# annalam/seqkit

Measured on AMD Instinct MI355X. Metric: M reads/s demultiplex (150bp, 96 barcodes) at 1/8 GPUs; % HBM roofline, higher is better.
Workload: dtype u8

## Files before the change

### seqkit_amd/build.py

```python
from __future__ import annotations

import os
import shutil
import subprocess
import sys

ROOT = os.path.dirname(os.path.abspath(__file__))
REPO = os.path.dirname(ROOT)
CSRC = os.path.join(ROOT, "csrc")
LIBDIR = os.path.join(ROOT, "lib")
BINDIR = os.path.join(ROOT, "bin")
LIB_PATH = os.path.join(LIBDIR, "libseqkit_hip.so")

HIP_SOURCES = ["sk_kernels.hip", "sk_census.hip", "sk_inflate.hip", "sk_deflate.hip", "sk_bamtext.hip", "sk_bamwrite.hip", "sk_bamminimize.hip", "sk_bammarkdup.hip", "sk_bamsubsample.hip", "sk_bammerge.hip", "sk_bamcoverage.hip", "sk_bampair.hip", "sk_bamtarget.hip", "sk_capi.hip", "sk_bamfile.cpp", "sk_bamfile_reads.cpp", "sk_bamfile_out.cpp", "sk_bamfile_coverage.cpp", "sk_lut.cpp"]
HIP_DEPS = HIP_SOURCES + ["sk_internal.h", "sk_lut.h", "sk_bamblock.h", "sk_bamfmt.h", "sk_bamfile.h", "sk_passmem.h", "sk_hoststage.h", os.path.join(REPO, "include", "seqkit_hip.h")]
HIP_FLAGS = ["--offload-arch=gfx950", "-O3", "-std=c++17", "-fPIC", "-shared", "-Wall", "-Wno-unused-function"]


def library_inputs_digest() -> str:
    import hashlib
    h = hashlib.sha256()
    h.update(" ".join(HIP_FLAGS).encode())
    for d in HIP_DEPS:
        p = d if os.path.isabs(d) else os.path.join(CSRC, d)
        with open(p, "rb") as f:
            h.update(os.path.basename(p).encode() + b"\0" + f.read())
    return h.hexdigest()[:16]


def _hipcc() -> str:
# ... 60 lines not shown
```

### seqkit_amd/csrc/sk_capi.hip

```cpp
#include <hip/hip_runtime.h>
#include <rccl/rccl.h>
#include <dlfcn.h>
#include <unistd.h>

#include <algorithm>
#include <cstdarg>
#include <cstdio>
#include <cstdlib>
#include <cstring>
#include <mutex>
#include <string>
#include <unordered_set>
#include <vector>

#include "../../include/seqkit_hip.h"
#include "sk_internal.h"
#include "sk_hoststage.h"

struct sk_ctx {
	int device = 0;
	int n_cu = 256;
	hipStream_t stream = nullptr;
	hipStream_t stream2 = nullptr;
	hipEvent_t ev0 = nullptr, ev1 = nullptr, ev_pipe = nullptr;
// ... 7 lines not shown
	int bs_bytes = 0, bs_mm_off = 0, G = 0;
	uint8_t *d_nbr = nullptr;
	sk::LutDev nbr{};
	std::vector<uint8_t> sheet;
	bool nbr_tried = false;
	int64_t nbr_keys = 0, nbr_bytes = 0;
	int detail_mode = SK_DETAIL_FULL;
	unsigned long long *d_counts = nullptr;
	unsigned long long *d_counts_wide = nullptr;
	bool wide_dirty = false;
	unsigned long long *d_count_rep = nullptr;
	int count_rep_pitch = 0;
	size_t count_rep_set = 0;
	uint8_t *ws = nullptr;
	size_t ws_bytes = 0;
	sk::ManyBatch *many_pin = nullptr;
	hipEvent_t many_ev[8] = {nullptr, nullptr, nullptr, nullptr, nullptr, nullptr, nullptr, nullptr};
	int many_next = 0;
	const void *many_no_tab = nullptr;
	int many_no_stride = 0, many_no_detail = -1;
	struct Kept { void *p = nullptr; size_t cap = 0; bool pinned = false; } kept[sk::kKeepSlots];
	void *ext = nullptr;
	void (*ext_free)(void *) = nullptr;
	sk::Census *census = nullptr;
	ncclComm_t comm = nullptr;
	int comm_ranks = 0;
	uint8_t *d_genome = nullptr;
	int64_t genome_len = 0;
	int cnt_n_chr = 0;
	int64_t cnt_n_regions = 0;
	uint8_t *d_cnt = nullptr;
	int32_t *d_chr_off = nullptr, *d_ridx = nullptr;
	uint32_t *d_rstart = nullptr, *d_rend = nullptr, *d_rpmax = nullptr, *d_region_frags = nullptr;
	int ot_n_chr = 0;
	uint8_t *d_ot = nullptr;
	int32_t *d_ot_chr_off = nullptr;
	int64_t *d_ot_rstart = nullptr, *d_ot_rpmax = nullptr;
	unsigned long long *d_ot_counters = nullptr;
};

static thread_local std::string g_create_err;

static constexpr int kManySlots = 8, kManyMax = 256;

static int fail(sk_ctx *c, int code, const char *fmt, ...)
{
	char buf[512];
	va_list ap;
	va_start(ap, fmt);
	vsnprintf(buf, sizeof buf, fmt, ap);
	va_end(ap);
	if (c) c->err = buf; else g_create_err = buf;
	return code;
}

#define SK_HIP(c, call)                                                                            \
	do {                                                                                           \
		hipError_t e_ = (call);                                                                    \
		if (e_ != hipSuccess) return fail((c), SK_ERR_HIP, "%s: %s", #call, hipGetErrorString(e_)); \
// ... 161 lines not shown
	if (!c) return;
	(void)hipSetDevice(c->device);
	if (c->stream) (void)hipStreamSynchronize(c->stream);
	if (c->stream2) (void)hipStreamSynchronize(c->stream2);
	if (c->d_raw) (void)hipFree(c->d_raw);
	if (c->d_onehot) (void)hipFree(c->d_onehot);
	if (c->d_lut) (void)hipFree(c->d_lut);
	if (c->d_bs) (void)hipFree(c->d_bs);
	if (c->d_nbr) (void)hipFree(c->d_nbr);
	if (c->d_counts) (void)hipFree(c->d_counts);
	if (c->d_counts_wide) (void)hipFree(c->d_counts_wide);
	if (c->d_count_rep) (void)hipFree(c->d_count_rep);
	if (c->ws) (void)hipFree(c->ws);
	for (auto &k : c->kept) if (k.p) { if (k.pinned) (void)hipHostFree(k.p); else (void)hipFree(k.p); }
	if (c->ext && c->ext_free) c->ext_free(c->ext);
	if (c->many_pin) (void)hipHostFree(c->many_pin);
	for (hipEvent_t e : c->many_ev) if (e) (void)hipEventDestroy(e);
	if (c->census) sk::census_destroy(c->census);
	if (c->comm) (void)sk_comm_destroy(c);
	if (c->d_cnt) (void)hipFree(c->d_cnt);
	if (c->d_ot) (void)hipFree(c->d_ot);
	if (c->d_genome) (void)hipFree(c->d_genome);
	if (c->ev0) (void)hipEventDestroy(c->ev0);
	if (c->ev1) (void)hipEventDestroy(c->ev1);
	if (c->ev_pipe) (void)hipEventDestroy(c->ev_pipe);
	if (c->stream2) (void)hipStreamDestroy(c->stream2);
	if (c->stream) (void)hipStreamDestroy(c->stream);
	delete c;
}

const char *sk_last_error(const sk_ctx *c) { return c ? c->err.c_str() : g_create_err.c_str(); }

// ... 75 lines not shown

int sk_set_barcodes(sk_ctx *c, const uint8_t *table, int S, int L, int max_diff)
{
	if (!c) return SK_ERR_INVALID;
	if (S < 0 || S > SK_MAX_SAMPLES) return fail(c, SK_ERR_INVALID, "S = %d outside 0..%d", S, SK_MAX_SAMPLES);
	if (L < 0 || L > SK_MAX_BARCODE_LEN || (S > 0 && L == 0)) return fail(c, SK_ERR_INVALID, "L = %d outside 1..%d", L, SK_MAX_BARCODE_LEN);
	if (S > 0 && !table) return fail(c, SK_ERR_INVALID, "table is NULL");
	if (max_diff < 0 || max_diff > 255) return fail(c, SK_ERR_INVALID, "max_diff = %d outside 0..255", max_diff);
	if (int r = bind(c)) return r;
	SK_HIP(c, hipStreamSynchronize(c->stream));
	if (c->d_raw) { SK_HIP(c, hipFree(c->d_raw)); c->d_raw = nullptr; }
	if (c->d_onehot) { SK_HIP(c, hipFree(c->d_onehot)); c->d_onehot = nullptr; }
	if (c->d_lut) { SK_HIP(c, hipFree(c->d_lut)); c->d_lut = nullptr; }
	if (c->d_bs) { SK_HIP(c, hipFree(c->d_bs)); c->d_bs = nullptr; }
	if (c->d_nbr) { SK_HIP(c, hipFree(c->d_nbr)); c->d_nbr = nullptr; }
	c->many_no_tab = nullptr;
	c->nbr = sk::LutDev{};
	c->bs_bytes = c->bs_mm_off = c->G = 0;
	if (c->d_counts) { SK_HIP(c, hipFree(c->d_counts)); c->d_counts = nullptr; }
	if (c->d_counts_wide) { SK_HIP(c, hipFree(c->d_counts_wide)); c->d_counts_wide = nullptr; }
	c->wide_dirty = false;
	if (c->d_count_rep) { SK_HIP(c, hipFree(c->d_count_rep)); c->d_count_rep = nullptr; }
	c->have_table = false;
	c->S = S; c->L = L; c->max_diff = max_diff;
	c->W = (L + 3) / 4;

	SK_HIP(c, hipMalloc((void **)&c->d_raw, (size_t)S * L + 16));
	if (S > 0) SK_HIP(c, hipMemcpy(c->d_raw, table, (size_t)S * L, hipMemcpyHostToDevice));

	bool onehot_ok = S > 0 && L <= sk::kMaxOneHotLen && !getenv("SK_NO_ONEHOT");
	std::vector<uint8_t> lut((size_t)(L ? L : 1) * 256, 0x80);
// ... 438 lines not shown
	if (t.bc && t.counts_wide) c->wide_dirty = true;
	SK_HIP(c, sk::launch_tile_pass(t, c->n_cu, c->stream));
	return SK_OK;
}

static void one_mate(sk_fused_args &a, const uint8_t *seq, const uint8_t *qual, const uint16_t *len, int stride, int64_t n,
                     uint8_t min_baseq, uint8_t *out_seq, uint16_t *lowest_k);

int sk_fused_pass_many_dev(sk_ctx *c, const sk_fused_args *batches, int n_batches)
{
	if (!c) return SK_ERR_INVALID;
	if (n_batches < 0 || (n_batches > 0 && !batches)) return fail(c, SK_ERR_INVALID, "n_batches = %d", n_batches);
	if (n_batches == 0) return SK_OK;
	if (int r = bind(c)) return r;
	for (int i = 0; i < n_batches; i++) if (int r = check_fused(c, &batches[i], true)) return r;
	{
		bool same = n_batches >= 2;
		int64_t rows = 0;
		for (int i = 0; i < n_batches && same; i++) {
			const sk_fused_args &a = batches[i], &f = batches[0];
			bool mates = false;
			for (int m = 0; m < a.n_mates; m++) mates = mates || a.mate[m].out_seq || a.mate[m].lowest_k;
			same = !mates && a.bc && !a.counts && a.bc_stride == f.bc_stride && !a.lowest_diff == !f.lowest_diff && !a.first_idx == !f.first_idx && !a.last_idx == !f.last_idx;
			rows += ((a.n + 255) / 256) * 256;
		}
		if (const char *ev = getenv("SK_MANY_ONE_LAUNCH")) same = same && atoi(ev) != 0;
		const int want_detail_key = same ? ((batches[0].lowest_diff ? 1 : 0) | (batches[0].first_idx ? 2 : 0) | (batches[0].last_idx ? 4 : 0) | (c->detail_mode << 3)) : 0;
		if (same && c->many_no_tab && c->many_no_tab == (const void *)c->d_nbr && c->many_no_stride == batches[0].bc_stride && c->many_no_detail == want_detail_key && !getenv("SK_LUT_MANY_GATHER")) same = false;
		if (same && rows > 0 && rows < ((int64_t)1 << 31) && n_batches <= kManyMax) {
			if (int r = prepare_demux(c, &batches[0])) return r;
			if (!c->many_pin) {
				SK_HIP(c, hipHostMalloc((void **)&c->many_pin, kManySlots * kManyMax * sizeof(sk::ManyBatch), hipHostMallocDefault));
				for (int k = 0; k < kManySlots; k++) SK_HIP(c, hipEventCreateWithFlags(&c->many_ev[k], hipEventDisableTiming));
			}
			const int slot = c->many_next++ % kManySlots;
			SK_HIP(c, hipEventSynchronize(c->many_ev[slot]));
			sk::ManyBatch *hb = c->many_pin + (size_t)slot * kManyMax;
			int64_t q0 = 0;
			int nb = 0;
			for (int i = 0; i < n_batches; i++) {
				const sk_fused_args &a = batches[i];
				if (a.n == 0) continue;
				const int64_t r0 = q0 * 256;
				sk::ManyBatch &m = hb[nb++];
				m.bc = a.bc - r0 * a.bc_stride;
				m.assign = a.assign - r0;
				m.lowest_diff = a.lowest_diff ? a.lowest_diff - r0 : nullptr;
				m.first_idx = a.first_idx ? a.first_idx - r0 : nullptr;
				m.last_idx = a.last_idx ? a.last_idx - r0 : nullptr;
				m.row_end = (uint32_t)(r0 + a.n);
				q0 += (a.n + 255) / 256;
				m.q_end = (int32_t)q0;
			}
			if (nb > 0) {
				sk_fused_args first = batches[0];
				for (int i = 0; i < n_batches; i++) if (batches[i].n > 0) { first = batches[i]; break; }
				sk::TileArgs t = tile_args_of(c, &first);
				t.n = q0 * 256;
				t.many = hb; t.n_many = nb; t.many_quads = (int)q0;
				if (t.counts_wide) c->wide_dirty = true;
				const hipError_t e = sk::launch_tile_pass(t, c->n_cu, c->stream);
				SK_HIP(c, hipEventRecord(c->many_ev[slot], c->stream));
				if (e == hipSuccess) return SK_OK;
				if (e != hipErrorNotSupported) return fail(c, SK_ERR_HIP, "launch_tile_pass (many batches): %s", hipGetErrorString(e));
				(void)hipGetLastError();
				if (t.n >= 1500000) { c->many_no_tab = (const void *)c->d_nbr; c->many_no_stride = batches[0].bc_stride; c->many_no_detail = want_detail_key; }
			} else return SK_OK;
		}
	}
	bool two = n_batches >= 2;
	int two_mode = 1;
	if (const char *ev = getenv("SK_MANY_TWO_STREAMS")) { two_mode = atoi(ev); two = two && two_mode != 0; }
	for (int i = 0; i < n_batches && two; i++) {
		if (batches[i].bc == nullptr) continue;
		bool mates = false;
		for (int m = 0; m < batches[i].n_mates; m++) mates = mates || batches[i].mate[m].out_seq || batches[i].mate[m].lowest_k;
		if (two_mode < 2 || mates || batches[i].counts) { two = false; break; }
		if (int r = prepare_demux(c, &batches[i])) return r;
		const sk::TileArgs t = tile_args_of(c, &batches[i]);
		two = t.counts_wide != nullptr && sk::tile_pass_demux_by_table(t);
	}
	if (two) {
		SK_HIP(c, hipEventRecord(c->ev_pipe, c->stream));
		SK_HIP(c, hipStreamWaitEvent(c->stream2, c->ev_pipe, 0));
	}
	int k = 0;
	for (int i = 0; i < n_batches; i++) {
		const sk_fused_args *a = &batches[i];
		if (a->n == 0) continue;
		if (int r = prepare_demux(c, a)) return r;
		sk::TileArgs t = tile_args_of(c, a);
		if (t.bc && t.counts_wide) c->wide_dirty = true;
		SK_HIP(c, sk::launch_tile_pass(t, c->n_cu, (two && (k & 1)) ? c->stream2 : c->stream));
		k++;
	}
	if (two) {
		SK_HIP(c, hipEventRecord(c->ev_pipe, c->stream2));
		SK_HIP(c, hipStreamWaitEvent(c->stream, c->ev_pipe, 0));
	}
	return SK_OK;
}

// ... 943 lines not shown
```

### seqkit_amd/csrc/sk_internal.h

```cpp
#pragma once
#include <hip/hip_runtime.h>
#include <stdint.h>

#include "sk_lut.h"

namespace sk {

constexpr int kWave = 64;
constexpr int kTileRows = 64;
constexpr int kLdsPad = 16;
constexpr int kMaxTileStride = 960;
constexpr int kMaxOneHotLen = 32;
constexpr int kKeyBits = 11;
constexpr int kMaxLdsHist = 1024;
constexpr int kAssignNone = -1;
constexpr int kAssignAmbiguous = -2;

struct QualConsts {
	uint32_t cl2;
	uint32_t c72;
	int mode;
	int min_baseq;
};
QualConsts make_qual_consts(int min_baseq);
// ... 8 lines not shown

struct BarcodeDev {
	const uint8_t *raw;
	const uint32_t *onehot;
	const uint8_t *lut;
	const uint8_t *bs;
	int bs_bytes, bs_mm_off, G;
	int S, L, W, max_diff;
	LutDev nbr;
	unsigned long long *count_rep;
	int count_rep_pitch;
};
constexpr int kCountReplicas = 16;
constexpr int kMaxBitSlicedLen = 31;
constexpr int kMaxBitSlicedBytes = 24 * 1024;

struct ManyBatch {
	const uint8_t *bc;
	int32_t *assign;
	uint8_t *lowest_diff;
	int16_t *first_idx, *last_idx;
	uint32_t row_end;
	int32_t q_end;
};

struct TileArgs {
	int64_t n;
	int n_mates;
	int stride;
	QualConsts qc;
	MateDev mate[2];
	const uint8_t *bc;
	int bc_stride;
	BarcodeDev table;
	int32_t *assign;
	uint8_t *lowest_diff;
	int16_t *first_idx;
	int16_t *last_idx;
	int detail_matched;
	unsigned long long *counts;
	unsigned long long *counts_wide;
	int counts_wide_rows;
	const ManyBatch *many;
	int n_many, many_quads;
};
constexpr int kCountWideShift = 4;
constexpr int kCountDenseFrom = 160;
constexpr int kCountDenseRows = 512;
hipError_t launch_counts_fold_wide(unsigned long long *wide, int nc, int dense_rows, unsigned long long *counts, hipStream_t st);

struct BlockedArgs {
	const uint8_t *in;
	uint8_t *out;
	int64_t n;
	int n_mates, stride, bc_stride;
	int in_block, out_block;
	int in_qual[2], in_seq[2], in_len[2], in_bc;
	int out_seq[2], out_lowest_k[2], out_assign, out_lowest_diff, out_first_idx, out_last_idx;
	QualConsts qc;
	BarcodeDev table;
	unsigned long long *counts;
};
hipError_t launch_tile_blocked(const BlockedArgs &a, int n_cu, hipStream_t st);
bool blocked_shape_ok(const BlockedArgs &a);

hipError_t launch_tile_pass(const TileArgs &a, int n_cu, hipStream_t st);
bool tile_pass_fuses_demux(bool has_bc, bool any_mate, int stride, bool has_bitsliced, int G, int S, int bc_stride);
hipError_t launch_mask_flat(const uint8_t *seq, const uint8_t *qual, uint8_t *out, int64_t bytes,
                            const QualConsts &qc, int n_cu, hipStream_t st);
hipError_t launch_bam_flag_tlen(const uint16_t *flag, const int32_t *tid, const int32_t *mtid, const int32_t *tlen,
                                int64_t n, int32_t max_frag, unsigned long long *out, int want_counters, int want_hist,
                                int n_cu, hipStream_t st);

hipError_t launch_bam_fragments(const uint16_t *flag, const int32_t *tid, const int32_t *mtid, const int32_t *tlen, int64_t n,
                                int64_t min_size, int64_t max_size, uint8_t *keep_bits, unsigned long long *kept, int n_cu, hipStream_t st);

struct CountArgs {
	const uint16_t *flag;
	const uint8_t *mapq;
	const int32_t *tid, *mtid, *pos, *mpos, *tlen, *end_pos;
	int64_t n;
// ... 197 lines not shown
```

### seqkit_amd/csrc/sk_kernels.hip

```cpp
#include "sk_internal.h"

#include <cstdlib>
#include <mutex>
#include <vector>

namespace sk {

#ifndef SK_STRAGGLER_FROM
#define SK_STRAGGLER_FROM 6
#endif
#ifndef SK_STRAGGLER_ROWS
#define SK_STRAGGLER_ROWS 8
#endif
#ifndef SK_STRAGGLER_LEFT
#define SK_STRAGGLER_LEFT 6
#endif

typedef uint32_t u32;
typedef __attribute__((ext_vector_type(4))) uint32_t u32x4;
typedef __attribute__((ext_vector_type(2))) uint32_t u32x2;

typedef const __attribute__((address_space(4))) uint32_t *const_u32_ptr;

constexpr u32 kLo7 = 0x7f7f7f7fu;
// ... 725 lines not shown
#ifdef SK_ST_AUX
constexpr int kAuxStreamSt = SK_ST_AUX;
#else
constexpr int kAuxStreamSt = (SK_NT & 2) ? 2 : 0;
#endif

template <class T>
__device__ __forceinline__ const T __attribute__((address_space(4))) *kernel_args_now()
{
	u32 z;
	asm volatile("s_mov_b32 %0, 0" : "=s"(z));
	return reinterpret_cast<const T __attribute__((address_space(4))) *>(
		(const char __attribute__((address_space(4))) *)__builtin_amdgcn_kernarg_segment_ptr() + z);
}

__device__ __forceinline__ rsrc_t make_rsrc(const void *p, int64_t byte_off, int records)
{
	return __builtin_amdgcn_make_buffer_rsrc(const_cast<uint8_t *>(static_cast<const uint8_t *>(p)) + (p ? byte_off : 0), 0, p ? records : 0, 0x00020000);
}

template <int MODE, bool DEMUX, int SLOTS>
__global__ __launch_bounds__(256, SLOTS > 4 ? 2 : 4) void tile_pass_kernel(const TileArgs a, const LdsPlan lp)
{
	constexpr bool kTrimOnly = SLOTS == 10;
	const int lane = threadIdx.x & (kWave - 1);
	const int wave = __builtin_amdgcn_readfirstlane(threadIdx.x >> 6);
	const int nwave = blockDim.x >> 6;
	uint8_t *tile = sk_smem + lp.tiles_off + wave * lp.tile_slot + kLdsPad;
	u32 *hist = reinterpret_cast<u32 *>(sk_smem + lp.hist_off);
	if (DEMUX) stage_tables(a.table, lp, hist);
// ... 367 lines not shown
{
	typedef u32 u32x2_t __attribute__((ext_vector_type(2)));
	typedef u32 u32x3_t __attribute__((ext_vector_type(3)));
	static_assert(N >= 2 && N <= 6, "a key segment of one to five dwords and the dword behind it");
	if constexpr (N == 2) { const u32x2_t v = __builtin_amdgcn_raw_buffer_load_b64(rb, off, 0, kLutAux); d[0] = v[0]; d[1] = v[1]; }
	else if constexpr (N == 3) { const u32x3_t v = __builtin_amdgcn_raw_buffer_load_b96(rb, off, 0, kLutAux); d[0] = v[0]; d[1] = v[1]; d[2] = v[2]; }
	else {
		const u32x4 v = __builtin_amdgcn_raw_buffer_load_b128(rb, off, 0, kLutAux);
		d[0] = v[0]; d[1] = v[1]; d[2] = v[2]; d[3] = v[3];
		if constexpr (N == 5) d[4] = __builtin_amdgcn_raw_buffer_load_b32(rb, off + 16, 0, kLutAux);
		if constexpr (N == 6) { const u32x2_t w = __builtin_amdgcn_raw_buffer_load_b64(rb, off + 16, 0, kLutAux); d[4] = w[0]; d[5] = w[1]; }
	}
}


template <int W1, int W2, bool DIRECT, bool LDSTAB, bool DETAIL, bool PAIR = false, bool MANY = false>
__global__ __launch_bounds__(LDSTAB ? 1024 : 256) void demux_lut_kernel(const TileArgs a, const LdsPlan lp)
{
	typedef u32 u32x2_t __attribute__((ext_vector_type(2)));
	constexpr int W = W1 + W2;
	static_assert(W >= 1 && W <= 5 && (W2 == 0 || W2 == W1) && !(DIRECT && (W2 > 0 || W1 > 2)), "shape");
	static_assert(!PAIR || (W2 == W1 && W1 <= 2 && LDSTAB && !DIRECT), "the factored form: two halves of one or two dwords, tables in LDS");
	const int lane = threadIdx.x & (kWave - 1);
	const int wave = __builtin_amdgcn_readfirstlane(threadIdx.x >> 6);
	const int nwave = blockDim.x >> 6;
	u32 *hist = reinterpret_cast<u32 *>(sk_smem + lp.hist_off);
	const LutDev &t = a.table.nbr;
	const int S = a.table.S;
	const int64_t ntiles = MANY ? 4 * (int64_t)a.many_quads : (a.n + kTileRows - 1) / kTileRows;
	const int bstride = a.bc_stride;
	constexpr int kDepth = PAIR ? SK_LUT_PAIR_DEPTH : SK_LUT_DEPTH;
	static_assert(kDepth == 1 || kDepth == 2 || kDepth == 4, "a quad's four tiles take the register slots in turn");
	u32 raw[kDepth][W];
// ... 2 lines not shown
	const int rs = lane * bstride, rs2 = rs + t.sep_off + 1;
	const u32 sh1 = (u32)rs & 3u, sh2 = (u32)rs2 & 3u;
	const u32 sep_sel = 0x0c0c0c00u | (sh1 + (u32)(t.sep_off - 4 * (W1 - 1)));
	const int nt32 = (int)ntiles, last_rows = (int)(a.n - (ntiles - 1) * kTileRows);
	auto rows_of = [&](int ti) { return ti < nt32 - 1 ? kTileRows : (ti == nt32 - 1 ? last_rows : 0); };
	auto rows_many = [&](int ti, u32 row_end) {
		const int left = (int)(row_end - (u32)ti * (u32)kTileRows);
		return left <= 0 ? 0 : (left < kTileRows ? left : kTileRows);
	};
	struct BatchView { const uint8_t *bc; u32 row_end; int q_end; };
	int cb = 0, fb = 0;
	BatchView cv = {nullptr, 0u, 0}, fv = {nullptr, 0u, 0};
	int32_t *c_assign = nullptr;
	uint8_t *c_low = nullptr;
	int16_t *c_first = nullptr, *c_last = nullptr;
	auto view_of = [&](int i) { const ManyBatch &m = a.many[i]; return BatchView{m.bc, m.row_end, m.q_end}; };
	auto seek = [&](int gq, int &cur, BatchView &v) {
		bool moved = false;
		while (cur + 1 < a.n_many && gq >= v.q_end) { cur++; v = view_of(cur); moved = true; }
		return moved;
	};
	if (MANY) {
		cv = fv = view_of(0);
		c_assign = a.many[0].assign; c_low = a.many[0].lowest_diff; c_first = a.many[0].first_idx; c_last = a.many[0].last_idx;
	}
	int cur_quad = 0;
	auto fetch = [&](int ti, int s) {
		const bool mine = (ti >> 2) == cur_quad;
		const u32 m_end = mine ? cv.row_end : fv.row_end;
		const uint8_t *m_bc = mine ? cv.bc : fv.bc;
		const int rows = MANY ? rows_many(ti, m_end) : rows_of(ti);
		const rsrc_t rb = make_rsrc(MANY ? m_bc : a.bc, (int64_t)(rows ? ti : 0) * (kTileRows * bstride), (rows * bstride + 3) & ~3);
		if (DIRECT) {
			if (W == 2) {
				const u32x2_t v = __builtin_amdgcn_raw_buffer_load_b64(rb, lane * bstride, 0, kLutAux);
				raw[s][0] = v[0]; raw[s][W - 1] = v[1];
			} else {
				raw[s][0] = __builtin_amdgcn_raw_buffer_load_b32(rb, lane * bstride, 0, kLutAux);
			}
		} else {
			gather_dwords<W1 + 1>(rb, rs & ~3, g1[s]);
			if constexpr (W2 > 0) gather_dwords<W2 + 1>(rb, rs2 & ~3, g2[s]);
		}
	};
	const int qstep = (int)gridDim.x * nwave;
	int qb = (int)blockIdx.x * nwave + wave;
	if (MANY) { seek(qb, cb, cv); fb = cb; fv = cv; seek(qb + qstep, fb, fv); cur_quad = qb; if (cb != 0) { const ManyBatch &mb = a.many[cb]; c_assign = mb.assign; c_low = mb.lowest_diff; c_first = mb.first_idx; c_last = mb.last_idx; } }
	for (int s = 0; s < kDepth; s++) fetch(4 * qb + s, s);
	
	if (lp.use_lds_hist) for (int i = threadIdx.x; i < S + 3; i += blockDim.x) hist[i] = 0u;
	const int ltab_off = lp.tiles_off - lp.table_bytes;
	if (LDSTAB) {
		const int n16 = lp.table_bytes >> 4;
		for (int i0 = threadIdx.x; i0 < n16; i0 += 8 * (int)blockDim.x) {
			u32x4 tv[8];
#pragma unroll
			for (int j = 0; j < 8; j++) {
				const int i = i0 + j * (int)blockDim.x;
				if (i < n16) tv[j] = reinterpret_cast<const u32x4 *>(PAIR ? t.pair.tab : t.tab)[i];
			}
#pragma unroll
			for (int j = 0; j < 8; j++) {
// ... 19 lines not shown
	auto entry2_w1 = [&](u32 slot) {
		if (LDSTAB) return *reinterpret_cast<const u32 *>(sk_smem + ltab_off2 + 4 + (int)slot * 8);
		return t.tab[(size_t)(t.mask + 1) * 2 + (size_t)slot * 2 + 1];
	};
	const u32 idx_bits = (u32)__builtin_popcount(t.idx_mask);
	u32 n_total = 0;
	u32 *tp = reinterpret_cast<u32 *>(sk_smem + lp.tiles_off + wave * lp.tile_slot);
	const int nq32 = (nt32 + 3) >> 2;
	for (; qb < nq32; qb += qstep) {
		int code[4], dtot[4], dfirst[4], dlast[4];
		u32 q_row_end = (u32)a.n;
		int32_t *q_assign = a.assign;
		uint8_t *q_low = a.lowest_diff;
		int16_t *q_first = a.first_idx, *q_last = a.last_idx;
		if (MANY) {
			if (seek(qb, cb, cv)) { const ManyBatch &mb = a.many[cb]; c_assign = mb.assign; c_low = mb.lowest_diff; c_first = mb.first_idx; c_last = mb.last_idx; }
			cur_quad = qb;
			q_row_end = cv.row_end; q_assign = c_assign; q_low = c_low; q_first = c_first; q_last = c_last;
			seek(qb + qstep, fb, fv);
		}
#pragma unroll
		for (int j = 0; j < 4; j++) {
			constexpr int kD = kDepth;
			const int s = j % kD;
			const int ti = 4 * qb + j;
			const int rows = MANY ? rows_many(ti, q_row_end) : rows_of(ti);
			const bool active = lane < rows;
			const int nj = j + kD;
			const int tnext = nj < 4 ? 4 * qb + nj : 4 * (qb + qstep) + (nj - 4);
			u32 d[W];
			u32 sepbad = 0u;
// ... 108 lines not shown
					const int64_t rt = ro + kTileRows * j;
					__builtin_amdgcn_raw_buffer_store_b8((uint8_t)dtot[j], make_rsrc(q_low, rj ? rt : 0, rj), lane, 0, 0);
					__builtin_amdgcn_raw_buffer_store_b16((unsigned short)dfirst[j], make_rsrc(q_first, (rj ? rt : 0) * 2, rj * 2), lane * 2, 0, 0);
					__builtin_amdgcn_raw_buffer_store_b16((unsigned short)dlast[j], make_rsrc(q_last, (rj ? rt : 0) * 2, rj * 2), lane * 2, 0, 0);
				}
			}
		}
	}
	if (!a.counts_wide && !a.table.count_rep) lut_identified_from_hist(S, hist, lane);
	const WaveCounts wc = {n_total, 0u, 0u};
	if (a.counts_wide && a.counts_wide_rows) flush_counts(S, a.counts_wide + (size_t)(blockIdx.x % (unsigned)a.counts_wide_rows) * (S + 3), lp, hist, lane, wc, 0);
	else if (a.counts_wide) flush_counts(S, a.counts_wide + (((size_t)(blockIdx.x & (kCountReplicas - 1)) * (S + 3)) << kCountWideShift), lp, hist, lane, wc, kCountWideShift);
	else flush_counts_spread(a.table, a.counts, lp, hist, lane, wc);
}

template <bool LDSTAB, bool DETAIL, bool MANY = false>
__global__ __launch_bounds__(LDSTAB ? 1024 : 256) void demux_lut8x2_kernel(const TileArgs a, const LdsPlan lp)
{
	typedef u32 u32x2_t __attribute__((ext_vector_type(2)));
	constexpr int kRows = 2 * kTileRows;
	const int lane = threadIdx.x & (kWave - 1);
	const int wave = __builtin_amdgcn_readfirstlane(threadIdx.x >> 6);
	const int nwave = blockDim.x >> 6;
	u32 *hist = reinterpret_cast<u32 *>(sk_smem + lp.hist_off);
	const LutDev &t = a.table.nbr;
	const int S = a.table.S;
	const int64_t ntiles = MANY ? 2 * (int64_t)a.many_quads : (a.n + kRows - 1) / kRows;
	const int nt32 = (int)ntiles, last_rows = (int)(a.n - (ntiles - 1) * kRows);
	auto rows_of = [&](int ti) { return ti < nt32 - 1 ? kRows : (ti == nt32 - 1 ? last_rows : 0); };
	auto rows_many = [&](int ti, u32 row_end) {
		const int left = (int)(row_end - (u32)ti * (u32)kRows);
		return left <= 0 ? 0 : (left < kRows ? left : kRows);
	};
	struct BatchView { const uint8_t *bc; u32 row_end; int q_end; };
	int cb = 0, fb = 0;
	BatchView cv = {nullptr, 0u, 0}, fv = {nullptr, 0u, 0};
	int32_t *c_assign = nullptr;
	uint8_t *c_low = nullptr;
	int16_t *c_first = nullptr, *c_last = nullptr;
	auto view_of = [&](int i) { const ManyBatch &m = a.many[i]; return BatchView{m.bc, m.row_end, m.q_end}; };
	auto seek = [&](int gq, int &cur, BatchView &v) {
		bool moved = false;
		while (cur + 1 < a.n_many && gq >= v.q_end) { cur++; v = view_of(cur); moved = true; }
		return moved;
	};
	if (MANY) {
		cv = fv = view_of(0);
		c_assign = a.many[0].assign; c_low = a.many[0].lowest_diff; c_first = a.many[0].first_idx; c_last = a.many[0].last_idx;
	}
	constexpr int kDepth = 2;
	u32x4 raw[kDepth];
	auto fetch = [&](int ti, int s) {
		if (MANY) {
			const int rows = rows_many(ti, fv.row_end);
			raw[s] = __builtin_amdgcn_raw_buffer_load_b128(make_rsrc(fv.bc, (int64_t)(rows ? ti : 0) * (kRows * 8), rows * 8), lane * 16, 0, kLut8Aux);
			return;
		}
		const int rows = rows_of(ti);
		raw[s] = __builtin_amdgcn_raw_buffer_load_b128(make_rsrc(a.bc, (int64_t)(rows ? ti : 0) * (kRows * 8), rows * 8), lane * 16, 0, kLut8Aux);
	};
	const int qstep = (int)gridDim.x * nwave;
	int qb = (int)blockIdx.x * nwave + wave;
	if (MANY) seek(qb, fb, fv);
// ... 34 lines not shown
	auto entry2_w1 = [&](u32 slot) {
		if (LDSTAB) return *reinterpret_cast<const u32 *>(sk_smem + ltab_off2 + 4 + (int)slot * 8);
		return t.tab[(size_t)(t.mask + 1) * 2 + (size_t)slot * 2 + 1];
	};
	const u32 idx_bits = (u32)__builtin_popcount(t.idx_mask);
	u32 n_total = 0;
	u32 *tp = reinterpret_cast<u32 *>(sk_smem + lp.tiles_off + wave * lp.tile_slot);
	const int nq32 = (nt32 + 1) >> 1;
	for (; qb < nq32; qb += qstep) {
		int code[2][2], tot[2][2], first[2][2], last[2][2];
		u32 q_row_end = (u32)a.n;
		int32_t *q_assign = a.assign;
		uint8_t *q_low = a.lowest_diff;
		int16_t *q_first = a.first_idx, *q_last = a.last_idx;
		if (MANY) {
			if (seek(qb, cb, cv)) { const ManyBatch &mb = a.many[cb]; c_assign = mb.assign; c_low = mb.lowest_diff; c_first = mb.first_idx; c_last = mb.last_idx; }
			q_row_end = cv.row_end; q_assign = c_assign; q_low = c_low; q_first = c_first; q_last = c_last;
			seek(qb + qstep, fb, fv);
		}
#pragma unroll
		for (int s = 0; s < 2; s++) {
			const int ti = 2 * qb + s;
			const int rows = MANY ? rows_many(ti, q_row_end) : rows_of(ti);
			const u32x4 d = raw[s];
			fetch(2 * (qb + qstep) + s, s);
#pragma unroll
			for (int r = 0; r < 2; r++) {
				u32 c[5] = {0u, 0u, 0u, 0u, 0u};
#pragma unroll
				for (int w = 0; w < 2; w++) {
					c[w] = lut_classes(d[2 * r + w], t);
// ... 244 lines not shown
}

bool tile_pass_fuses_demux(bool has_bc, bool any_mate, int stride, bool has_bitsliced, int G, int S, int bc_stride)
{
	static const bool env_no_fuse = getenv("SK_NO_FUSED_DEMUX") != nullptr;
	return has_bc && any_mate && stride <= kMaxTileStride && has_bitsliced && G <= 4 && S > 0 && kTileRows * bc_stride <= 2048 && !env_no_fuse;
}

bool tile_pass_demux_by_table(const TileArgs &b)
{
	const bool env_no_hash = getenv("SK_NO_HASH_DEMUX") != nullptr;
	const bool want_detail = b.lowest_diff || b.first_idx || b.last_idx;
	return (b.table.nbr.tab || b.table.nbr.pair.tab) && (!want_detail || b.detail_matched) && kTileRows * b.bc_stride <= 2048 && !env_no_hash;
}

hipError_t launch_tile_pass(const TileArgs &a, int n_cu, hipStream_t st)
{
	if (a.n <= 0) return hipSuccess;
	if ((a.n + kTileRows - 1) / kTileRows > (int64_t)1 << 30) return hipErrorInvalidValue;
	TileArgs b = a;
	bool any_mate = false;
	for (int mi = 0; mi < b.n_mates; mi++) any_mate = any_mate || b.mate[mi].out_seq || b.mate[mi].lowest_k;
	if (any_mate && b.stride > kMaxTileStride) {
		for (int mi = 0; mi < b.n_mates; mi++) {
			MateDev &mt = b.mate[mi];
			if (mt.out_seq) {
				hipError_t e = launch_mask_flat(mt.seq, mt.qual, mt.out_seq, b.n * (int64_t)b.stride, b.qc, n_cu, st);
				if (e != hipSuccess) return e;
			}
			if (mt.lowest_k) {
				int64_t want = (b.n + 255) / 256;
				int grid = (int)(want < (int64_t)n_cu * 8 ? want : (int64_t)n_cu * 8);
				trim_rows_global_kernel<<<grid, 256, 0, st>>>(mt.qual, mt.len, b.stride, b.n, b.qc.min_baseq, mt.lowest_k);
				hipError_t e = hipGetLastError();
				if (e != hipSuccess) return e;
			}
			mt.out_seq = nullptr; mt.lowest_k = nullptr;
		}
		any_mate = false;
	}
	const bool fuse_demux = tile_pass_fuses_demux(b.bc != nullptr, any_mate, b.stride, b.table.bs != nullptr, b.table.G, b.table.S, b.bc_stride);
	if (b.bc && !fuse_demux) {
		const bool env_no_hash = getenv("SK_NO_HASH_DEMUX") != nullptr;
		const bool want_detail = b.lowest_diff || b.first_idx || b.last_idx;
		const bool by_table = tile_pass_demux_by_table(b);
		hipError_t e;
		TileArgs bb = b;
		if (b.many && !by_table) return hipErrorNotSupported;
		if (by_table) {
			const LutDev &t = b.table.nbr;
			const bool pair = t.pair.tab != nullptr;
			const char *env_direct = getenv("SK_DEMUX_DIRECT");
			const bool direct = !pair && (b.bc_stride & 3) == 0 && t.W2 == 0 && t.W1 <= 2 && 4 * t.W1 <= b.bc_stride && (!env_direct || atoi(env_direct) != 0);
			const char *env_ldstab = getenv("SK_DEMUX_LDSTAB");
			const int table_bytes = pair ? t.pair.bytes : (t.mask + 1) * 2 * 8;
			const bool ldstab = pair || (table_bytes <= (128 << 10) && (!env_ldstab || atoi(env_ldstab) != 0));
			const char *env_rows2 = getenv("SK_DEMUX_ROWS2");
			const bool rows2 = direct && t.W1 == 2 && b.bc_stride == 8 && (env_rows2 ? atoi(env_rows2) != 0 : (want_detail || b.n >= 1500000));
			const void *fn = pair ? (t.W1 == 1 ? (want_detail ? reinterpret_cast<const void *>(demux_lut_kernel<1, 1, false, true, true, true>) : reinterpret_cast<const void *>(demux_lut_kernel<1, 1, false, true, false, true>))
			                                   : (want_detail ? reinterpret_cast<const void *>(demux_lut_kernel<2, 2, false, true, true, true>) : reinterpret_cast<const void *>(demux_lut_kernel<2, 2, false, true, false, true>)))
			                 : rows2 ? (ldstab ? (want_detail ? reinterpret_cast<const void *>(demux_lut8x2_kernel<true, true>) : reinterpret_cast<const void *>(demux_lut8x2_kernel<true, false>))
			                                 : (want_detail ? reinterpret_cast<const void *>(demux_lut8x2_kernel<false, true>) : reinterpret_cast<const void *>(demux_lut8x2_kernel<false, false>)))
			                 : ldstab ? (want_detail ? demux_lut_fn<true, true>(t.W1, t.W2, direct) : demux_lut_fn<true, false>(t.W1, t.W2, direct))
			                          : (want_detail ? demux_lut_fn<false, true>(t.W1, t.W2, direct) : demux_lut_fn<false, false>(t.W1, t.W2, direct));
			if (b.many) {
				if (!ldstab) return hipErrorNotSupported;
				const char *mg = getenv("SK_LUT_MANY_GATHER");
				const bool many_gather = mg && atoi(mg) != 0;
				if (rows2) fn = want_detail ? reinterpret_cast<const void *>(demux_lut8x2_kernel<true, true, true>) : reinterpret_cast<const void *>(demux_lut8x2_kernel<true, false, true>);
				else if (many_gather && !direct && t.W1 == 2 && t.W2 == 2)
					fn = pair ? (want_detail ? reinterpret_cast<const void *>(demux_lut_kernel<2, 2, false, true, true, true, true>) : reinterpret_cast<const void *>(demux_lut_kernel<2, 2, false, true, false, true, true>))
					          : (want_detail ? reinterpret_cast<const void *>(demux_lut_kernel<2, 2, false, true, true, false, true>) : reinterpret_cast<const void *>(demux_lut_kernel<2, 2, false, true, false, false, true>));
				else return hipErrorNotSupported;
			}
			LdsPlan lp{};
			lp.use_lds_hist = 1;
			lp.hist_off = 0;
			lp.table_bytes = ldstab ? table_bytes : 0;
			lp.tiles_off = (((b.table.S + 3) * 4 + 15) & ~15) + lp.table_bytes;
			lp.tile_slot = 4 * kTileRows * 4;
			int nw = ldstab ? ((lp.table_bytes > (64 << 10) && b.n >= 4000000) ? 8 : 16) : 4;
			static const int env_nw = [] { const char *v = getenv("SK_LUT_NW"); return v ? atoi(v) : 0; }();
			static const int env_wg = [] { const char *v = getenv("SK_LUT_WG"); return v ? atoi(v) : 0; }();
			if (env_nw >= 1 && env_nw <= (ldstab ? 16 : 4)) nw = env_nw;
			while (nw > 4 && lp.tiles_off + nw * lp.tile_slot > 160 * 1024) nw >>= 1;
			const int lds = lp.tiles_off + nw * lp.tile_slot;
			struct Occ { int dev; const void *fn; int lds, nw, wg; };
// ... 5 lines not shown
			{
				std::lock_guard<std::mutex> lk(occ_m);
				for (const Occ &o : occ) if (o.dev == dev && o.fn == fn && o.lds == lds && o.nw == nw) wg = o.wg;
			}
			if (wg == 0) {
				e = hipFuncSetAttribute(fn, hipFuncAttributeMaxDynamicSharedMemorySize, 160 * 1024);
				if (e == hipSuccess) e = hipOccupancyMaxActiveBlocksPerMultiprocessor(&wg, fn, kWave * nw, (size_t)lds);
				if (e != hipSuccess) return e;
				if (wg < 1) return hipErrorInvalidValue;
				std::lock_guard<std::mutex> lk(occ_m);
				occ.push_back({dev, fn, lds, nw, wg});
			}
			if (ldstab && wg > 1) wg = 1;
			if (env_wg >= 1) wg = env_wg;
			const int tile_rows = 4 * kTileRows;
			const int64_t ntiles = b.many ? (int64_t)b.many_quads : (b.n + tile_rows - 1) / tile_rows, want = (ntiles + nw - 1) / nw, cap = (int64_t)n_cu * wg;
			const int64_t grid = want < cap ? want : cap;
			if (grid <= 512 || bb.counts_wide) bb.table.count_rep = nullptr;
			void *kargs[] = {(void *)&bb, (void *)&lp};
			e = hipLaunchKernel(fn, dim3((unsigned)grid), dim3(kWave * nw), kargs, lds, st);
		} else {
			e = plan_and_launch(reinterpret_cast<const void *>(demux_tile_kernel), b, b.bc_stride, true, 4, n_cu, st);
		}
		if (e == hipSuccess && !(by_table && bb.counts_wide)) e = launch_counts_fold(bb, by_table, st);
		if (e != hipSuccess) return e;
	}
	if (!any_mate) return hipSuccess;
	int row_bytes = 0;
	for (int mi = 0; mi < b.n_mates; mi++)
		if (b.mate[mi].lowest_k) row_bytes = b.stride;
	const int64_t total = b.n * (int64_t)b.stride;
	if (total & 3)
		for (int mi = 0; mi < b.n_mates; mi++)
			if (b.mate[mi].out_seq) mask_tail_kernel<<<1, 4, 0, st>>>(b.mate[mi].seq, b.mate[mi].qual, b.mate[mi].out_seq, total, b.qc.min_baseq);
// ... 653 lines not shown
```

Measured before the change: 6714.

## Pass many-batch descriptors inline via kernel arguments instead of pinned host ring

The per-batch descriptor table for the multi-batch demux launch is now packed into a ManyBatchSet of up to 32 entries and passed inline in the kernel argument segment. This replaces the pinned host buffer with its event ring and the per-call event synchronisation. Large request lists are split into several launches of up to 32 batches each. The gather path (SK_LUT_MANY_GATHER) is now on by default, and the negative cache that disabled the single-launch path after a failure is removed. The trade-offs are a larger kernarg block per launch and extra launches when there are more than 32 batches.

```diff
diff --git a/seqkit_amd/build.py b/seqkit_amd/build.py
--- a/seqkit_amd/build.py
+++ b/seqkit_amd/build.py
@@ -13,7 +13,7 @@
 LIB_PATH = os.path.join(LIBDIR, "libseqkit_hip.so")
 
 HIP_SOURCES = ["sk_kernels.hip", "sk_census.hip", "sk_inflate.hip", "sk_deflate.hip", "sk_bamtext.hip", "sk_bamwrite.hip", "sk_bamminimize.hip", "sk_bammarkdup.hip", "sk_bamsubsample.hip", "sk_bammerge.hip", "sk_bamcoverage.hip", "sk_bampair.hip", "sk_bamtarget.hip", "sk_capi.hip", "sk_bamfile.cpp", "sk_bamfile_reads.cpp", "sk_bamfile_out.cpp", "sk_bamfile_coverage.cpp", "sk_lut.cpp"]
-HIP_DEPS = HIP_SOURCES + ["sk_internal.h", "sk_lut.h", "sk_bamblock.h", "sk_bamfmt.h", "sk_bamfile.h", "sk_passmem.h", "sk_hoststage.h", os.path.join(REPO, "include", "seqkit_hip.h")]
+HIP_DEPS = HIP_SOURCES + ["sk_internal.h", "sk_manypack.h", "sk_lut.h", "sk_bamblock.h", "sk_bamfmt.h", "sk_bamfile.h", "sk_passmem.h", "sk_hoststage.h", os.path.join(REPO, "include", "seqkit_hip.h")]
 HIP_FLAGS = ["--offload-arch=gfx950", "-O3", "-std=c++17", "-fPIC", "-shared", "-Wall", "-Wno-unused-function"]
 
 
diff --git a/seqkit_amd/csrc/sk_capi.hip b/seqkit_amd/csrc/sk_capi.hip
--- a/seqkit_amd/csrc/sk_capi.hip
+++ b/seqkit_amd/csrc/sk_capi.hip
@@ -45,11 +45,6 @@
 	size_t count_rep_set = 0;
 	uint8_t *ws = nullptr;
 	size_t ws_bytes = 0;
-	sk::ManyBatch *many_pin = nullptr;
-	hipEvent_t many_ev[8] = {nullptr, nullptr, nullptr, nullptr, nullptr, nullptr, nullptr, nullptr};
-	int many_next = 0;
-	const void *many_no_tab = nullptr;
-	int many_no_stride = 0, many_no_detail = -1;
 	struct Kept { void *p = nullptr; size_t cap = 0; bool pinned = false; } kept[sk::kKeepSlots];
 	void *ext = nullptr;
 	void (*ext_free)(void *) = nullptr;
@@ -72,8 +67,6 @@
 
 static thread_local std::string g_create_err;
 
-static constexpr int kManySlots = 8, kManyMax = 256;
-
 static int fail(sk_ctx *c, int code, const char *fmt, ...)
 {
 	char buf[512];
@@ -265,8 +258,6 @@
 	if (c->ws) (void)hipFree(c->ws);
 	for (auto &k : c->kept) if (k.p) { if (k.pinned) (void)hipHostFree(k.p); else (void)hipFree(k.p); }
 	if (c->ext && c->ext_free) c->ext_free(c->ext);
-	if (c->many_pin) (void)hipHostFree(c->many_pin);
-	for (hipEvent_t e : c->many_ev) if (e) (void)hipEventDestroy(e);
 	if (c->census) sk::census_destroy(c->census);
 	if (c->comm) (void)sk_comm_destroy(c);
 	if (c->d_cnt) (void)hipFree(c->d_cnt);
@@ -372,7 +363,6 @@
 	if (c->d_lut) { SK_HIP(c, hipFree(c->d_lut)); c->d_lut = nullptr; }
 	if (c->d_bs) { SK_HIP(c, hipFree(c->d_bs)); c->d_bs = nullptr; }
 	if (c->d_nbr) { SK_HIP(c, hipFree(c->d_nbr)); c->d_nbr = nullptr; }
-	c->many_no_tab = nullptr;
 	c->nbr = sk::LutDev{};
 	c->bs_bytes = c->bs_mm_off = c->G = 0;
 	if (c->d_counts) { SK_HIP(c, hipFree(c->d_counts)); c->d_counts = nullptr; }
@@ -841,58 +831,42 @@
 	if (n_batches == 0) return SK_OK;
 	if (int r = bind(c)) return r;
 	for (int i = 0; i < n_batches; i++) if (int r = check_fused(c, &batches[i], true)) return r;
+	int loop_from = 0;
 	{
 		bool same = n_batches >= 2;
-		int64_t rows = 0;
 		for (int i = 0; i < n_batches && same; i++) {
 			const sk_fused_args &a = batches[i], &f = batches[0];
 			bool mates = false;
 			for (int m = 0; m < a.n_mates; m++) mates = mates || a.mate[m].out_seq || a.mate[m].lowest_k;
 			same = !mates && a.bc && !a.counts && a.bc_stride == f.bc_stride && !a.lowest_diff == !f.lowest_diff && !a.first_idx == !f.first_idx && !a.last_idx == !f.last_idx;
-			rows += ((a.n + 255) / 256) * 256;
 		}
 		if (const char *ev = getenv("SK_MANY_ONE_LAUNCH")) same = same && atoi(ev) != 0;
-		const int want_detail_key = same ? ((batches[0].lowest_diff ? 1 : 0) | (batches[0].first_idx ? 2 : 0) | (batches[0].last_idx ? 4 : 0) | (c->detail_mode << 3)) : 0;
-		if (same && c->many_no_tab && c->many_no_tab == (const void *)c->d_nbr && c->many_no_stride == batches[0].bc_stride && c->many_no_detail == want_detail_key && !getenv("SK_LUT_MANY_GATHER")) same = false;
-		if (same && rows > 0 && rows < ((int64_t)1 << 31) && n_batches <= kManyMax) {
+		if (same) {
 			if (int r = prepare_demux(c, &batches[0])) return r;
-			if (!c->many_pin) {
-				SK_HIP(c, hipHostMalloc((void **)&c->many_pin, kManySlots * kManyMax * sizeof(sk::ManyBatch), hipHostMallocDefault));
-				for (int k = 0; k < kManySlots; k++) SK_HIP(c, hipEventCreateWithFlags(&c->many_ev[k], hipEventDisableTiming));
-			}
-			const int slot = c->many_next++ % kManySlots;
-			SK_HIP(c, hipEventSynchronize(c->many_ev[slot]));
-			sk::ManyBatch *hb = c->many_pin + (size_t)slot * kManyMax;
-			int64_t q0 = 0;
-			int nb = 0;
-			for (int i = 0; i < n_batches; i++) {
+			const auto batch_of = [&](int i) {
 				const sk_fused_args &a = batches[i];
-				if (a.n == 0) continue;
-				const int64_t r0 = q0 * 256;
-				sk::ManyBatch &m = hb[nb++];
-				m.bc = a.bc - r0 * a.bc_stride;
-				m.assign = a.assign - r0;
-				m.lowest_diff = a.lowest_diff ? a.lowest_diff - r0 : nullptr;
-				m.first_idx = a.first_idx ? a.first_idx - r0 : nullptr;
-				m.last_idx = a.last_idx ? a.last_idx - r0 : nullptr;
-				m.row_end = (uint32_t)(r0 + a.n);
-				q0 += (a.n + 255) / 256;
-				m.q_end = (int32_t)q0;
-			}
-			if (nb > 0) {
-				sk_fused_args first = batches[0];
-				for (int i = 0; i < n_batches; i++) if (batches[i].n > 0) { first = batches[i]; break; }
-				sk::TileArgs t = tile_args_of(c, &first);
-				t.n = q0 * 256;
-				t.many = hb; t.n_many = nb; t.many_quads = (int)q0;
+				return sk::ManyIn{a.bc, a.n, a.bc_stride, a.assign, a.lowest_diff, a.first_idx, a.last_idx};
+			};
+			sk::ManyBatchSet set;
+			int next = 0;
+			for (;;) {
+				const int from = next;
+				const int64_t steps = sk::many_pack_next(batch_of, n_batches, &next, &set);
+				if (steps == 0) return SK_OK;
+				loop_from = from;
+				if (steps < 0) break;
+				int i0 = from;
+				while (batches[i0].n == 0) i0++;
+				sk::TileArgs t = tile_args_of(c, &batches[i0]);
+				t.n = steps * sk::kManyStepRows;
+				t.many_quads = (int)steps;
 				if (t.counts_wide) c->wide_dirty = true;
-				const hipError_t e = sk::launch_tile_pass(t, c->n_cu, c->stream);
-				SK_HIP(c, hipEventRecord(c->many_ev[slot], c->stream));
-				if (e == hipSuccess) return SK_OK;
+				const hipError_t e = sk::launch_tile_pass(t, c->n_cu, c->stream, &set);
+				if (e == hipSuccess) continue;
 				if (e != hipErrorNotSupported) return fail(c, SK_ERR_HIP, "launch_tile_pass (many batches): %s", hipGetErrorString(e));
 				(void)hipGetLastError();
-				if (t.n >= 1500000) { c->many_no_tab = (const void *)c->d_nbr; c->many_no_stride = batches[0].bc_stride; c->many_no_detail = want_detail_key; }
-			} else return SK_OK;
+				break;
+			}
 		}
 	}
 	bool two = n_batches >= 2;
@@ -912,7 +886,7 @@
 		SK_HIP(c, hipStreamWaitEvent(c->stream2, c->ev_pipe, 0));
 	}
 	int k = 0;
-	for (int i = 0; i < n_batches; i++) {
+	for (int i = loop_from; i < n_batches; i++) {
 		const sk_fused_args *a = &batches[i];
 		if (a->n == 0) continue;
 		if (int r = prepare_demux(c, a)) return r;
diff --git a/seqkit_amd/csrc/sk_internal.h b/seqkit_amd/csrc/sk_internal.h
--- a/seqkit_amd/csrc/sk_internal.h
+++ b/seqkit_amd/csrc/sk_internal.h
@@ -3,6 +3,7 @@
 #include <stdint.h>
 
 #include "sk_lut.h"
+#include "sk_manypack.h"
 
 namespace sk {
 
@@ -46,15 +47,6 @@
 constexpr int kCountReplicas = 16;
 constexpr int kMaxBitSlicedLen = 31;
 constexpr int kMaxBitSlicedBytes = 24 * 1024;
-
-struct ManyBatch {
-	const uint8_t *bc;
-	int32_t *assign;
-	uint8_t *lowest_diff;
-	int16_t *first_idx, *last_idx;
-	uint32_t row_end;
-	int32_t q_end;
-};
 
 struct TileArgs {
 	int64_t n;
@@ -73,8 +65,7 @@
 	unsigned long long *counts;
 	unsigned long long *counts_wide;
 	int counts_wide_rows;
-	const ManyBatch *many;
-	int n_many, many_quads;
+	int many_quads;
 };
 constexpr int kCountWideShift = 4;
 constexpr int kCountDenseFrom = 160;
@@ -96,7 +87,7 @@
 hipError_t launch_tile_blocked(const BlockedArgs &a, int n_cu, hipStream_t st);
 bool blocked_shape_ok(const BlockedArgs &a);
 
-hipError_t launch_tile_pass(const TileArgs &a, int n_cu, hipStream_t st);
+hipError_t launch_tile_pass(const TileArgs &a, int n_cu, hipStream_t st, const ManyBatchSet *many = nullptr);
 bool tile_pass_fuses_demux(bool has_bc, bool any_mate, int stride, bool has_bitsliced, int G, int S, int bc_stride);
 hipError_t launch_mask_flat(const uint8_t *seq, const uint8_t *qual, uint8_t *out, int64_t bytes,
                             const QualConsts &qc, int n_cu, hipStream_t st);
diff --git a/seqkit_amd/csrc/sk_kernels.hip b/seqkit_amd/csrc/sk_kernels.hip
--- a/seqkit_amd/csrc/sk_kernels.hip
+++ b/seqkit_amd/csrc/sk_kernels.hip
@@ -763,6 +763,15 @@
 		(const char __attribute__((address_space(4))) *)__builtin_amdgcn_kernarg_segment_ptr() + z);
 }
 
+constexpr unsigned kManyArgOffset = (unsigned)((((sizeof(TileArgs) + alignof(LdsPlan) - 1) / alignof(LdsPlan) * alignof(LdsPlan) + sizeof(LdsPlan)) + alignof(ManyBatchSet) - 1)
+                                               / alignof(ManyBatchSet) * alignof(ManyBatchSet));
+static_assert(kManyArgOffset + sizeof(ManyBatchSet) <= 4096, "the kernel arguments of a many-batch launch fit the 4 KiB argument segment");
+typedef const ManyBatchSet __attribute__((address_space(4))) *many_set_ptr;
+__device__ __forceinline__ many_set_ptr many_set_arg()
+{
+	return reinterpret_cast<many_set_ptr>((const char __attribute__((address_space(4))) *)__builtin_amdgcn_kernarg_segment_ptr() + kManyArgOffset);
+}
+
 __device__ __forceinline__ rsrc_t make_rsrc(const void *p, int64_t byte_off, int records)
 {
 	return __builtin_amdgcn_make_buffer_rsrc(const_cast<uint8_t *>(static_cast<const uint8_t *>(p)) + (p ? byte_off : 0), 0, p ? records : 0, 0x00020000);
@@ -1160,9 +1169,11 @@
 }
 
 
-template <int W1, int W2, bool DIRECT, bool LDSTAB, bool DETAIL, bool PAIR = false, bool MANY = false>
-__global__ __launch_bounds__(LDSTAB ? 1024 : 256) void demux_lut_kernel(const TileArgs a, const LdsPlan lp)
-{
+template <int W1, int W2, bool DIRECT, bool LDSTAB, bool DETAIL, bool PAIR = false, bool MANY = false, class... MS>
+__global__ __launch_bounds__(LDSTAB ? 1024 : 256) void demux_lut_kernel(const TileArgs a, const LdsPlan lp, const MS...)
+{
+	static_assert(sizeof...(MS) == (MANY ? 1 : 0), "the MANY forms take the batches' ManyBatchSet, the others nothing");
+	const many_set_ptr ms = many_set_arg();
 	typedef u32 u32x2_t __attribute__((ext_vector_type(2)));
 	constexpr int W = W1 + W2;
 	static_assert(W >= 1 && W <= 5 && (W2 == 0 || W2 == W1) && !(DIRECT && (W2 > 0 || W1 > 2)), "shape");
@@ -1195,15 +1206,17 @@
 	int32_t *c_assign = nullptr;
 	uint8_t *c_low = nullptr;
 	int16_t *c_first = nullptr, *c_last = nullptr;
-	auto view_of = [&](int i) { const ManyBatch &m = a.many[i]; return BatchView{m.bc, m.row_end, m.q_end}; };
+	const int n_many = MANY ? ms->n : 0;
+	auto outputs_of = [&](int i) { c_assign = ms->b[i].assign; c_low = ms->b[i].lowest_diff; c_first = ms->b[i].first_idx; c_last = ms->b[i].last_idx; };
+	auto view_of = [&](int i) { return BatchView{ms->b[i].bc, ms->b[i].row_end, ms->b[i].q_end}; };
 	auto seek = [&](int gq, int &cur, BatchView &v) {
 		bool moved = false;
-		while (cur + 1 < a.n_many && gq >= v.q_end) { cur++; v = view_of(cur); moved = true; }
+		while (cur + 1 < n_many && gq >= v.q_end) { cur++; v = view_of(cur); moved = true; }
 		return moved;
 	};
 	if (MANY) {
 		cv = fv = view_of(0);
-		c_assign = a.many[0].assign; c_low = a.many[0].lowest_diff; c_first = a.many[0].first_idx; c_last = a.many[0].last_idx;
+		outputs_of(0);
 	}
 	int cur_quad = 0;
 	auto fetch = [&](int ti, int s) {
@@ -1226,7 +1239,7 @@
 	};
 	const int qstep = (int)gridDim.x * nwave;
 	int qb = (int)blockIdx.x * nwave + wave;
-	if (MANY) { seek(qb, cb, cv); fb = cb; fv = cv; seek(qb + qstep, fb, fv); cur_quad = qb; if (cb != 0) { const ManyBatch &mb = a.many[cb]; c_assign = mb.assign; c_low = mb.lowest_diff; c_first = mb.first_idx; c_last = mb.last_idx; } }
+	if (MANY) { seek(qb, cb, cv); fb = cb; fv = cv; seek(qb + qstep, fb, fv); cur_quad = qb; if (cb != 0) outputs_of(cb); }
 	for (int s = 0; s < kDepth; s++) fetch(4 * qb + s, s);
 	
 	if (lp.use_lds_hist) for (int i = threadIdx.x; i < S + 3; i += blockDim.x) hist[i] = 0u;
@@ -1276,7 +1289,7 @@
 		uint8_t *q_low = a.lowest_diff;
 		int16_t *q_first = a.first_idx, *q_last = a.last_idx;
 		if (MANY) {
-			if (seek(qb, cb, cv)) { const ManyBatch &mb = a.many[cb]; c_assign = mb.assign; c_low = mb.lowest_diff; c_first = mb.first_idx; c_last = mb.last_idx; }
+			if (seek(qb, cb, cv)) outputs_of(cb);
 			cur_quad = qb;
 			q_row_end = cv.row_end; q_assign = c_assign; q_low = c_low; q_first = c_first; q_last = c_last;
 			seek(qb + qstep, fb, fv);
@@ -1415,9 +1428,11 @@
 	else flush_counts_spread(a.table, a.counts, lp, hist, lane, wc);
 }
 
-template <bool LDSTAB, bool DETAIL, bool MANY = false>
-__global__ __launch_bounds__(LDSTAB ? 1024 : 256) void demux_lut8x2_kernel(const TileArgs a, const LdsPlan lp)
-{
+template <bool LDSTAB, bool DETAIL, bool MANY = false, class... MS>
+__global__ __launch_bounds__(LDSTAB ? 1024 : 256) void demux_lut8x2_kernel(const TileArgs a, const LdsPlan lp, const MS...)
+{
+	static_assert(sizeof...(MS) == (MANY ? 1 : 0), "the MANY forms take the batches' ManyBatchSet, the others nothing");
+	const many_set_ptr ms = many_set_arg();
 	typedef u32 u32x2_t __attribute__((ext_vector_type(2)));
 	constexpr int kRows = 2 * kTileRows;
 	const int lane = threadIdx.x & (kWave - 1);
@@ -1439,15 +1454,17 @@
 	int32_t *c_assign = nullptr;
 	uint8_t *c_low = nullptr;
 	int16_t *c_first = nullptr, *c_last = nullptr;
-	auto view_of = [&](int i) { const ManyBatch &m = a.many[i]; return BatchView{m.bc, m.row_end, m.q_end}; };
+	const int n_many = MANY ? ms->n : 0;
+	auto outputs_of = [&](int i) { c_assign = ms->b[i].assign; c_low = ms->b[i].lowest_diff; c_first = ms->b[i].first_idx; c_last = ms->b[i].last_idx; };
+	auto view_of = [&](int i) { return BatchView{ms->b[i].bc, ms->b[i].row_end, ms->b[i].q_end}; };
 	auto seek = [&](int gq, int &cur, BatchView &v) {
 		bool moved = false;
-		while (cur + 1 < a.n_many && gq >= v.q_end) { cur++; v = view_of(cur); moved = true; }
+		while (cur + 1 < n_many && gq >= v.q_end) { cur++; v = view_of(cur); moved = true; }
 		return moved;
 	};
 	if (MANY) {
 		cv = fv = view_of(0);
-		c_assign = a.many[0].assign; c_low = a.many[0].lowest_diff; c_first = a.many[0].first_idx; c_last = a.many[0].last_idx;
+		outputs_of(0);
 	}
 	constexpr int kDepth = 2;
 	u32x4 raw[kDepth];
@@ -1512,7 +1529,7 @@
 		uint8_t *q_low = a.lowest_diff;
 		int16_t *q_first = a.first_idx, *q_last = a.last_idx;
 		if (MANY) {
-			if (seek(qb, cb, cv)) { const ManyBatch &mb = a.many[cb]; c_assign = mb.assign; c_low = mb.lowest_diff; c_first = mb.first_idx; c_last = mb.last_idx; }
+			if (seek(qb, cb, cv)) outputs_of(cb);
 			q_row_end = cv.row_end; q_assign = c_assign; q_low = c_low; q_first = c_first; q_last = c_last;
 			seek(qb + qstep, fb, fv);
 		}
@@ -1787,9 +1804,10 @@
 	return (b.table.nbr.tab || b.table.nbr.pair.tab) && (!want_detail || b.detail_matched) && kTileRows * b.bc_stride <= 2048 && !env_no_hash;
 }
 
-hipError_t launch_tile_pass(const TileArgs &a, int n_cu, hipStream_t st)
+hipError_t launch_tile_pass(const TileArgs &a, int n_cu, hipStream_t st, const ManyBatchSet *many)
 {
 	if (a.n <= 0) return hipSuccess;
+	if ((a.many_quads > 0) != (many != nullptr) || (many && (many->n < 1 || many->n > kManyInline))) return hipErrorInvalidValue;
 	if ((a.n + kTileRows - 1) / kTileRows > (int64_t)1 << 30) return hipErrorInvalidValue;
 	TileArgs b = a;
 	bool any_mate = false;
@@ -1819,7 +1837,7 @@
 		const bool by_table = tile_pass_demux_by_table(b);
 		hipError_t e;
 		TileArgs bb = b;
-		if (b.many && !by_table) return hipErrorNotSupported;
+		if (many && !by_table) return hipErrorNotSupported;
 		if (by_table) {
 			const LutDev &t = b.table.nbr;
 			const bool pair = t.pair.tab != nullptr;
@@ -1836,14 +1854,14 @@
 			                                 : (want_detail ? reinterpret_cast<const void *>(demux_lut8x2_kernel<false, true>) : reinterpret_cast<const void *>(demux_lut8x2_kernel<false, false>)))
 			                 : ldstab ? (want_detail ? demux_lut_fn<true, true>(t.W1, t.W2, direct) : demux_lut_fn<true, false>(t.W1, t.W2, direct))
 			                          : (want_detail ? demux_lut_fn<false, true>(t.W1, t.W2, direct) : demux_lut_fn<false, false>(t.W1, t.W2, direct));
-			if (b.many) {
+			if (many) {
 				if (!ldstab) return hipErrorNotSupported;
 				const char *mg = getenv("SK_LUT_MANY_GATHER");
-				const bool many_gather = mg && atoi(mg) != 0;
-				if (rows2) fn = want_detail ? reinterpret_cast<const void *>(demux_lut8x2_kernel<true, true, true>) : reinterpret_cast<const void *>(demux_lut8x2_kernel<true, false, true>);
+				const bool many_gather = !mg || atoi(mg) != 0;
+				if (rows2) fn = want_detail ? reinterpret_cast<const void *>(demux_lut8x2_kernel<true, true, true, ManyBatchSet>) : reinterpret_cast<const void *>(demux_lut8x2_kernel<true, false, true, ManyBatchSet>);
 				else if (many_gather && !direct && t.W1 == 2 && t.W2 == 2)
-					fn = pair ? (want_detail ? reinterpret_cast<const void *>(demux_lut_kernel<2, 2, false, true, true, true, true>) : reinterpret_cast<const void *>(demux_lut_kernel<2, 2, false, true, false, true, true>))
-					          : (want_detail ? reinterpret_cast<const void *>(demux_lut_kernel<2, 2, false, true, true, false, true>) : reinterpret_cast<const void *>(demux_lut_kernel<2, 2, false, true, false, false, true>));
+					fn = pair ? (want_detail ? reinterpret_cast<const void *>(demux_lut_kernel<2, 2, false, true, true, true, true, ManyBatchSet>) : reinterpret_cast<const void *>(demux_lut_kernel<2, 2, false, true, false, true, true, ManyBatchSet>))
+					          : (want_detail ? reinterpret_cast<const void *>(demux_lut_kernel<2, 2, false, true, true, false, true, ManyBatchSet>) : reinterpret_cast<const void *>(demux_lut_kernel<2, 2, false, true, false, false, true, ManyBatchSet>));
 				else return hipErrorNotSupported;
 			}
 			LdsPlan lp{};
@@ -1879,10 +1897,10 @@
 			if (ldstab && wg > 1) wg = 1;
 			if (env_wg >= 1) wg = env_wg;
 			const int tile_rows = 4 * kTileRows;
-			const int64_t ntiles = b.many ? (int64_t)b.many_quads : (b.n + tile_rows - 1) / tile_rows, want = (ntiles + nw - 1) / nw, cap = (int64_t)n_cu * wg;
+			const int64_t ntiles = many ? (int64_t)b.many_quads : (b.n + tile_rows - 1) / tile_rows, want = (ntiles + nw - 1) / nw, cap = (int64_t)n_cu * wg;
 			const int64_t grid = want < cap ? want : cap;
 			if (grid <= 512 || bb.counts_wide) bb.table.count_rep = nullptr;
-			void *kargs[] = {(void *)&bb, (void *)&lp};
+			void *kargs[] = {(void *)&bb, (void *)&lp, (void *)many};
 			e = hipLaunchKernel(fn, dim3((unsigned)grid), dim3(kWave * nw), kargs, lds, st);
 		} else {
 			e = plan_and_launch(reinterpret_cast<const void *>(demux_tile_kernel), b, b.bc_stride, true, 4, n_cu, st);
diff --git a/seqkit_amd/csrc/sk_manypack.h b/seqkit_amd/csrc/sk_manypack.h
--- /dev/null
+++ b/seqkit_amd/csrc/sk_manypack.h
@@ -0,0 +1,68 @@
+#pragma once
+#include <stdint.h>
+
+namespace sk {
+
+struct ManyBatch {
+	const uint8_t *bc;
+	int32_t *assign;
+	uint8_t *lowest_diff;
+	int16_t *first_idx, *last_idx;
+	uint32_t row_end;
+	int32_t q_end;
+};
+
+constexpr int kManyInline = 32;
+struct ManyBatchSet {
+	int n;
+	ManyBatch b[kManyInline];
+};
+
+struct ManyIn {
+	const uint8_t *bc;
+	int64_t n;
+	int stride;
+	int32_t *assign;
+	uint8_t *lowest_diff;
+	int16_t *first_idx, *last_idx;
+};
+
+constexpr int64_t kManyStepRows = 256;
+constexpr int64_t kManyMaxSteps = (((int64_t)1 << 31) - 1) / kManyStepRows;
+
+template <class Get>
+inline int64_t many_pack_next(Get get, int n, int *next, ManyBatchSet *set)
+{
+	int i = *next;
+	while (i < n && get(i).n <= 0) i++;
+	*next = i;
+	if (i == n) return 0;
+	int64_t q0 = 0;
+	int nb = 0;
+	for (; i < n && nb < kManyInline; i++) {
+		const ManyIn a = get(i);
+		if (a.n <= 0) continue;
+		const int64_t steps = (a.n + kManyStepRows - 1) / kManyStepRows;
+		if (steps > kManyMaxSteps - q0) {
+			if (nb == 0) return -1;
+			break;
+		}
+		const uint64_t r0 = (uint64_t)(q0 * kManyStepRows);
+		auto biased = [&](const void *p, uint64_t elem_bytes) { return p ? (uintptr_t)p - (uintptr_t)(r0 * elem_bytes) : (uintptr_t)0; };
+		ManyBatch &m = set->b[nb++];
+		m.bc = reinterpret_cast<const uint8_t *>(biased(a.bc, (uint64_t)a.stride));
+		m.assign = reinterpret_cast<int32_t *>(biased(a.assign, 4));
+		m.lowest_diff = reinterpret_cast<uint8_t *>(biased(a.lowest_diff, 1));
+		m.first_idx = reinterpret_cast<int16_t *>(biased(a.first_idx, 2));
+		m.last_idx = reinterpret_cast<int16_t *>(biased(a.last_idx, 2));
+		m.row_end = (uint32_t)(r0 + (uint64_t)a.n);
+		q0 += steps;
+		m.q_end = (int32_t)q0;
+	}
+	while (i < n && get(i).n <= 0) i++;
+	*next = i;
+	set->n = nb;
+	return q0;
+}
+
+}
```

Measured after the change: 6707. Within noise of the previous version (-0.1%).
